# BadgerTechnologies/navigation

Hardware: AMD Instinct MI355X
Metric: scored trajectories/sec (whole node) + costmap inflation cells/sec, 400x400 map (higher is better)
Workload: dtype f64

## Files before the change

include/navgpu.h:

```cpp
#ifndef NAVGPU_H_
#define NAVGPU_H_

#include <stddef.h>
#include <stdint.h>

#ifdef __cplusplus
extern "C" {
#endif

typedef enum {
  NAVGPU_OK = 0,
  NAVGPU_ERR_INVALID = -1,
  NAVGPU_ERR_NO_DEVICE = -2,
  NAVGPU_ERR_HIP = -3,
  NAVGPU_ERR_CAPACITY = -4,
  NAVGPU_ERR_STATE = -5
} navgpu_status;

#define NAVGPU_NO_INFORMATION 255
#define NAVGPU_LETHAL_OBSTACLE 254
#define NAVGPU_INSCRIBED_INFLATED_OBSTACLE 253
#define NAVGPU_FREE_SPACE 0

#define NAVGPU_LAYER_STATIC 1
// ... 151 lines not shown
int navgpu_footprint_from_radius(double radius, double* xy16);
int navgpu_set_footprint(navgpu_fleet* fleet, uint32_t first, uint32_t count, const double* footprint_xy,
                         uint32_t n_vertices);

int navgpu_costmap_stage(navgpu_fleet* fleet, uint32_t first, uint32_t count, const double* robot_poses,
                         const navgpu_observation* observations, uint32_t n_observations,
                         const float* points_xyz, uint32_t n_points_total);
int navgpu_costmap_update(navgpu_fleet* fleet, uint32_t first, uint32_t count);
int navgpu_costmap_bounds(navgpu_fleet* fleet, uint32_t first, uint32_t count, int32_t* boxes);

int navgpu_inflate(navgpu_fleet* fleet, uint32_t first, uint32_t count, const int32_t* boxes);
int navgpu_obstacle_update_bounds(navgpu_fleet* fleet, uint32_t first, uint32_t count, double* bounds_inout);
int navgpu_obstacle_update_costs(navgpu_fleet* fleet, uint32_t first, uint32_t count, const int32_t* boxes);

int navgpu_planner_configure(navgpu_fleet* fleet, const navgpu_dwa_config* config);
int navgpu_planner_set_plan(navgpu_fleet* fleet, uint32_t first, uint32_t count);
int navgpu_planner_stage(navgpu_fleet* fleet, uint32_t first, uint32_t count, const navgpu_robot_state* states,
                         const double* plan_xy, uint32_t n_plan_total);
int navgpu_planner_stage_poses(navgpu_fleet* fleet, uint32_t first, uint32_t count, const float* pos_xyth, const float* vel_xyth);
int navgpu_planner_cycle(navgpu_fleet* fleet, uint32_t first, uint32_t count);
int navgpu_planner_set_bounded_map_grids(navgpu_fleet* fleet, int32_t enable);
int navgpu_planner_set_map_grid_options(navgpu_fleet* fleet, int32_t critic, int32_t aggregation, double yshift);
int navgpu_planner_wavefront_levels(navgpu_fleet* fleet, uint32_t first, uint32_t count, uint32_t* levels);
int navgpu_planner_wavefront_boxes(navgpu_fleet* fleet, uint32_t first, uint32_t count, int32_t* boxes);
int navgpu_planner_results(navgpu_fleet* fleet, uint32_t first, uint32_t count, navgpu_plan_result* results);
int navgpu_planner_set_cycles_in_flight(navgpu_fleet* fleet, int32_t cycles);
int navgpu_planner_results_previous(navgpu_fleet* fleet, uint32_t first, uint32_t count, navgpu_plan_result* results);
int navgpu_planner_trajectory(navgpu_fleet* fleet, uint32_t instance, double* xyth, uint32_t capacity_points);
int navgpu_planner_samples(navgpu_fleet* fleet, uint32_t instance, double* costs, int32_t* status,
                           float* velocities_xyz, uint32_t capacity);
int navgpu_planner_check_trajectory(navgpu_fleet* fleet, uint32_t instance, const float vel_samples[3], int32_t* ok);
int navgpu_planner_check_trajectories(navgpu_fleet* fleet, uint32_t n_robots, const uint32_t* instances,
                                      const uint32_t* probe_offsets , const float* vel_samples ,
                                      int32_t* ok , double* costs );
int navgpu_planner_cost_cloud(navgpu_fleet* fleet, uint32_t instance, float* points, uint32_t capacity);
#define NAVGPU_TRAJ_CLOUD_MAX_ROBOTS 16
int navgpu_planner_set_trajectory_cloud(navgpu_fleet* fleet, uint32_t first, uint32_t count, int32_t enable);
int navgpu_planner_trajectory_cloud(navgpu_fleet* fleet, uint32_t instance, int32_t reference_costs, float* points, uint32_t capacity);
typedef struct {
  double critic[5];
  double cost_full;
  double cost_ref;
  int32_t first_fail;
  int32_t status;
  int32_t n_points;
  int32_t member;
// ... 575 lines not shown
```

navigation_amd/_lib.py:

```python
import ctypes as C
import os
import subprocess

import numpy as np

_HERE = os.path.dirname(os.path.abspath(__file__))
_LIB = None

LAYER_STATIC, LAYER_OBSTACLE, LAYER_VOXEL, LAYER_INFLATION = 1, 2, 4, 8
GRID_MASTER, GRID_STATIC, GRID_OBSTACLE, GRID_VOXEL, GRID_PATH, GRID_GOAL, GRID_GOAL_FRONT = range(7)
OBS_MARKING, OBS_CLEARING = 1, 2
VOXEL_UNKNOWN, VOXEL_MARKED = 1, 2
K_OBSTACLE, K_MERGE, K_INFLATE, K_BFS, K_SCORE, K_SELECT, K_FOOTPRINT, K_VOXEL_EXPORT, K_OBS_INGEST, K_CHECK_TRAJ = range(10)
KERNELS = ("k_obstacle", "k_merge", "k_inflate", "k_bfs", "k_score", "k_select", "k_footprint_cost", "k_voxel_export", "k_obs_ingest", "k_check_traj")
CLOUD_XYZ, CLOUD_SCAN = 0, 1
OBSBUF_MAX_SOURCES, OBSBUF_MAX_CLOUD_POINTS = 8, 65536


class NavgpuError(RuntimeError):
    pass


class FleetDesc(C.Structure):
    _fields_ = [("n_instances", C.c_uint32), ("size_x", C.c_uint32), ("size_y", C.c_uint32),
# ... 414 lines not shown
    ("navgpu_grid_reset", C.c_int, [vp, C.c_int, u32, u32]),
    ("navgpu_grid_reset_window", C.c_int, [vp, C.c_int, u32, u32, u32, u32, u32, u32]),
    ("navgpu_layer_reset_bounding_box", C.c_int, [vp, u32, u32, vp]),
    ("navgpu_static_set_map", C.c_int, [vp, u32, u32, vp, i32, i32, i32, i32, i32]),
    ("navgpu_static_set_rolling_map", C.c_int, [vp, vp, u32, u32, C.c_double, C.c_double, C.c_double, i32, i32, i32, i32, i32]),
    ("navgpu_static_set_transform", C.c_int, [vp, u32, u32, vp]),
    ("navgpu_obstacle_configure", C.c_int, [vp, C.POINTER(ObstacleParams)]),
    ("navgpu_inflation_configure", C.c_int, [vp, C.POINTER(InflationParams)]),
    ("navgpu_set_footprint", C.c_int, [vp, u32, u32, vp, u32]),
    ("navgpu_costmap_stage", C.c_int, [vp, u32, u32, vp, vp, u32, vp, u32]),
    ("navgpu_costmap_update", C.c_int, [vp, u32, u32]),
    ("navgpu_costmap_bounds", C.c_int, [vp, u32, u32, vp]),
    ("navgpu_inflate", C.c_int, [vp, u32, u32, vp]),
    ("navgpu_obstacle_update_bounds", C.c_int, [vp, u32, u32, vp]),
    ("navgpu_obstacle_update_costs", C.c_int, [vp, u32, u32, vp]),
    ("navgpu_planner_configure", C.c_int, [vp, C.POINTER(DwaConfig)]),
    ("navgpu_planner_set_plan", C.c_int, [vp, u32, u32]),
    ("navgpu_planner_stage", C.c_int, [vp, u32, u32, vp, vp, u32]),
    ("navgpu_planner_stage_poses", C.c_int, [vp, u32, u32, vp, vp]),
    ("navgpu_planner_cycle", C.c_int, [vp, u32, u32]),
    ("navgpu_planner_set_bounded_map_grids", C.c_int, [vp, C.c_int32]),
    ("navgpu_planner_set_map_grid_options", C.c_int, [vp, C.c_int32, C.c_int32, C.c_double]),
    ("navgpu_planner_wavefront_levels", C.c_int, [vp, u32, u32, vp]),
    ("navgpu_planner_wavefront_boxes", C.c_int, [vp, u32, u32, vp]),
    ("navgpu_planner_results", C.c_int, [vp, u32, u32, vp]),
    ("navgpu_planner_set_cycles_in_flight", C.c_int, [vp, C.c_int32]),
    ("navgpu_planner_results_previous", C.c_int, [vp, u32, u32, vp]),
    ("navgpu_planner_trajectory", C.c_int, [vp, u32, vp, u32]),
    ("navgpu_planner_samples", C.c_int, [vp, u32, vp, vp, vp, u32]),
    ("navgpu_planner_check_trajectory", C.c_int, [vp, u32, vp, C.POINTER(i32)]),
    ("navgpu_planner_check_trajectories", C.c_int, [vp, u32, vp, vp, vp, vp, vp]),
    ("navgpu_planner_cost_cloud", C.c_int, [vp, u32, vp, u32]),
    ("navgpu_planner_set_trajectory_cloud", C.c_int, [vp, u32, u32, i32]),
    ("navgpu_planner_trajectory_cloud", C.c_int, [vp, u32, i32, vp, u32]),
    ("navgpu_planner_sample_terms", C.c_int, [vp, u32, vp, u32]),
    ("navgpu_planner_get_oscillation", C.c_int, [vp, u32, u32, vp, vp]),
    ("navgpu_planner_set_oscillation", C.c_int, [vp, u32, u32, vp, vp]),
    ("navgpu_local_plan_window", C.c_int, [vp, u32, vp, vp, dbl, i32, vp, u32, C.POINTER(u32), C.POINTER(u32)]),
    ("navgpu_shortest_angular_distance", dbl, [dbl, dbl]),
    ("navgpu_local_planner_configure", C.c_int, [vp, C.POINTER(LocalLimits)]),
    ("navgpu_local_planner_set_plan", C.c_int, [vp, u32, vp, u32, vp]),
    ("navgpu_local_planner_compute_velocity_commands", C.c_int, [vp, u32, u32, vp, vp]),
    ("navgpu_local_planner_is_goal_reached", C.c_int, [vp, u32, u32, vp, vp]),
    ("navgpu_local_planner_get_plan", C.c_int, [vp, u32, vp, u32]),
    ("navgpu_local_planner_reserve_plans", C.c_int, [vp, u32]),
    ("navgpu_local_planner_set_plans", C.c_int, [vp, u32, u32, vp, vp, vp]),
# ... 134 lines not shown
```

navigation_amd/csrc/navgpu_device.h:

```cpp
#pragma once
#include <hip/hip_runtime.h>
#include <stdint.h>

#include "../../include/navgpu.h"

namespace navgpu {

constexpr uint8_t kNoInfo = 255, kLethal = 254, kInscribed = 253, kFree = 0;
constexpr int kMaxFootprint = 32;
constexpr int kCareRows = 128, kCareWords = 4;
#ifndef NAVGPU_SCORE_TAB_THREADS
#define NAVGPU_SCORE_TAB_THREADS 256
#endif
#ifndef NAVGPU_SCORE_TAB_LDS_KB
#define NAVGPU_SCORE_TAB_LDS_KB 14
#endif
#ifndef NAVGPU_SCORE_PREP_THREADS
#define NAVGPU_SCORE_PREP_THREADS 256
#endif
#ifndef NAVGPU_SCORE_THREADS
#define NAVGPU_SCORE_THREADS 256
#endif
#ifdef NAVGPU_DEBUG_SWITCHES
#define NAVGPU_DEBUG_ENV(name) getenv(name)
#else
#define NAVGPU_DEBUG_ENV(name) ((const char*)nullptr)
#endif
constexpr int kScoreThreads = NAVGPU_SCORE_THREADS;

struct InstCostmapState {
  double last_min_x, last_min_y, last_max_x, last_max_y;
  int32_t need_reinflation;
  int32_t static_has_updated_data;
// ... 92 lines not shown
  uint32_t* within;
  uint32_t win;
  uint32_t fp_rcells;
  uint8_t fp_halfw[32];
  uint32_t fp_chunk;
  uint32_t use_tables, tab_steps, tab_nfp, tab_nth;
  int32_t mg_agg[4];
  double mg_yshift[4];
  int32_t mg_generic;
  uint32_t tab_rows;
  uint32_t tab_bytes;
  double tab_dt;
  uint8_t* prep;
  uint32_t prep_stride, prep_bytes;
  double* sample_cost;
  int32_t* sample_status;
  double* part_cost;
  int32_t* part_index;
  int32_t* counters;
  uint32_t* osc_flags;
  float* osc_prev;
  navgpu_plan_result* result;
  double* traj;
};

struct SampleTerms {
  double v[5];
  int32_t first_fail;
  int32_t fail_code;
  int32_t status;
  int32_t n_points;
};
static_assert(sizeof(SampleTerms) == 56, "terms record");
struct TrajCloudDev {
  const SampleTerms* terms;
  navgpu_sample_terms* out;
  uint32_t* totals;
  float* points;
  uint32_t capacity;
  uint32_t slots_per_group;
  double scale[5];
  int32_t reference_costs;
};
void launch_score_terms(const PlannerDev& pl, uint32_t inst, SampleTerms* terms, hipStream_t s);
struct ProbeBatch {
  const uint32_t* instances;
// ... 324 lines not shown
```

navigation_amd/csrc/navgpu_host.cpp:

```cpp
#include "navgpu_fleet.h"

namespace navgpu {
thread_local std::string g_last_error;
}

extern "C" {

const char* navgpu_version(void) { return "navgpu 0.1 (gfx950)"; }
const char* navgpu_strerror(int status) {
  switch (status) {
    case NAVGPU_OK: return "ok";
    case NAVGPU_ERR_INVALID: return "invalid argument";
    case NAVGPU_ERR_NO_DEVICE: return "no usable HIP device (this library has no CPU fallback)";
    case NAVGPU_ERR_HIP: return "HIP runtime error";
    case NAVGPU_ERR_CAPACITY: return "input exceeds a capacity given at fleet creation";
    case NAVGPU_ERR_STATE: return "call sequence violated";
    default: return "unknown status";
  }
}
const char* navgpu_last_error(void) { return g_last_error.c_str(); }
int navgpu_device_count(void) {
  int n = 0;
  if (hipGetDeviceCount(&n) != hipSuccess) return 0;
  return n;
// ... 173 lines not shown
    f->hp_state = reinterpret_cast<navgpu_robot_state*>(h + o_state);
    f->hp_front = reinterpret_cast<double*>(h + o_front);
    f->hp_align = reinterpret_cast<int32_t*>(h + o_align);
    f->hp_reach = reinterpret_cast<uint32_t*>(h + o_reach);
    f->hp_plan_cnt = reinterpret_cast<uint32_t*>(h + o_pcnt);
    f->hp_plan = reinterpret_cast<double*>(h + o_plan);
  }
  A(pl.fp_spec, (size_t)n * kMaxFootprint * 2);
  A(pl.fp_n, n);
  A(pl.axis_count, (size_t)n * 4);
  A(pl.path, (size_t)n * pl.cells);
  A(pl.goal, (size_t)n * pl.cells);
  A(pl.goal_front, (size_t)n * pl.cells);
  if (bfs_scratch_words(cm.nx, cm.ny)) A(pl.bfs_scratch, (size_t)n * bfs_scratch_words(cm.nx, cm.ny));
  pl.bfs_grids = 3;
  pl.within = nullptr;
  A(pl.bfs_box, (size_t)n * 8);
  A(pl.bfs_care, (size_t)n * kCareRows * kCareWords);
  A(pl.bfs_next_item, 4);
  A(pl.bfs_free, (size_t)n * cm.ny * ((cm.nx + 31) / 32));
  A(pl.bfs_levels, (size_t)n * 3);
  A(pl.bfs_order, (size_t)n * 3);
  pl.bfs_bounded = 0;
  A(pl.counters, (size_t)n * 2);
  A(pl.osc_flags, n);
  A(pl.osc_prev, (size_t)n * 3);
  A(pl.traj, (size_t)n * pl.max_sim_steps * 3);
#undef A
  f->h_origin.assign((size_t)n * 2, 0.0);
  f->h_fp_spec.assign((size_t)n * kMaxFootprint * 2, 0.0);
  f->h_fp_n.assign(n, 0);
  f->grid_partial.assign(n, 0);
  f->obs_consumed.assign(n, 0);
  f->bounded_grids = true;
  f->h_box.assign((size_t)n * 4, 0);
  f->inputs_gen.assign(n, 0);
  f->cycle_gen.assign(n, 0);
  launch_fill_u8(cm.master, cm.master_default, (size_t)n * cm.cells_padded, f->stream);
  if (cm.obst) launch_fill_u8(cm.obst, cm.obstacle_default, (size_t)n * cm.cells_padded, f->stream);
  if (cm.voxel) launch_fill_u32(cm.voxel, 0x0000FFFFu, (size_t)n * cm.cells_padded, f->stream);
  std::vector<InstCostmapState> st(n);
  for (auto& s : st) {
    memset(&s, 0, sizeof(s));
    s.last_min_x = -FLT_MAX;
    s.last_min_y = -FLT_MAX;
    s.last_max_x = FLT_MAX;
// ... 825 lines not shown
  if (f->cycles_in_flight > 1) {
    HIP_TRY(hipEventRecord(f->ev_pl_h2d, f->stream));
    f->ev_pl_set = true;
  }
  return NAVGPU_OK;
}

int navgpu_planner_set_bounded_map_grids(navgpu_fleet* f, int32_t enable) {
  if (!f) return NAVGPU_ERR_INVALID;
  FleetGuard guard_(f);
  f->bounded_grids = enable != 0;
  return restageReach(f);
}
int navgpu_planner_set_map_grid_options(navgpu_fleet* f, int32_t critic, int32_t aggregation, double yshift) {
  if (!f || critic < 0 || critic > 3 || aggregation < 0 || aggregation > 2 || !std::isfinite(yshift)) return NAVGPU_ERR_INVALID;
  FleetGuard guard_(f);
  PlannerDev& pl = f->pl;
  pl.mg_agg[critic] = aggregation;
  pl.mg_yshift[critic] = yshift;
  pl.mg_generic = 0;
  for (int k = 0; k < 4; ++k)
    if (pl.mg_agg[k] != 0 || pl.mg_yshift[k] != 0.0) pl.mg_generic = 1;
  return restageReach(f);
}
int navgpu_planner_wavefront_levels(navgpu_fleet* f, uint32_t first, uint32_t count, uint32_t* levels) {
  if (!f || !levels || !f->rangeOk(first, count)) return NAVGPU_ERR_INVALID;
  FleetGuard guard_(f);
  HIP_TRY(hipMemcpyAsync(levels, f->pl.bfs_levels + (size_t)first * 3, sizeof(uint32_t) * 3 * count, hipMemcpyDeviceToHost, f->stream));
  HIP_TRY(waitStream(f->stream));
  return NAVGPU_OK;
}

int navgpu_planner_configure(navgpu_fleet* f, const navgpu_dwa_config* c) {
  if (!f || !c) return NAVGPU_ERR_INVALID;
  FleetGuard guard_(f);
  if (!(c->sim_time > 0) || !(c->sim_granularity > 0) || !(c->angular_sim_granularity > 0)) return NAVGPU_ERR_INVALID;
  PlannerDev& pl = f->pl;
  navgpu_dwa_config cfg = *c;
  if (cfg.vx_samples <= 0) cfg.vx_samples = 1;
  if (cfg.vy_samples <= 0) cfg.vy_samples = 1;
  if (cfg.vth_samples <= 0) cfg.vth_samples = 1;
  if (cfg.rollout_trig != 0 && cfg.rollout_trig != 1) return NAVGPU_ERR_INVALID;
  const uint32_t max_axis = (uint32_t)std::max(std::max(cfg.vx_samples, cfg.vy_samples), std::max(cfg.vth_samples, 2)) + 1;
  if (max_axis > 128) return NAVGPU_ERR_CAPACITY;
  double steps;
  if (cfg.discretize_by_time)
// ... 544 lines not shown
```

navigation_amd/csrc/planner_bfs_common.h:

```cpp
#pragma once
#include "planner_common.h"

namespace navgpu {

template <typename Set>
__device__ __forceinline__ void bfsPlanSeeds(const PlannerDev& pl, const uint32_t inst, const int which, const Geom& g, const uint8_t* master,
                                             const uint32_t nx, const uint32_t tid, uint32_t* s_wave, Set&& set) {
  const uint32_t n = pl.plan_count[inst];
  const double* P = pl.plan + (size_t)inst * pl.max_plan * 2;
  const bool ovr = which == 2;
  const double lx = pl.front_last[2 * inst], ly = pl.front_last[2 * inst + 1];
  const uint32_t chunk = (n + blockDim.x - 1) / blockDim.x;
  const uint32_t i0 = min(n, tid * chunk), i1 = min(n, i0 + chunk);
  uint32_t mine = 0;
  for (uint32_t i = i0; i < i1; ++i) mine += adjustedPoints(P, i, lx, ly, ovr, n, g.res, true, [](uint32_t, double, double) {});
  uint32_t total;
  const uint32_t base = blockExclusiveScan1024(mine, s_wave, &total);
  auto valid = [&](double x, double y, uint32_t& cell) {
    uint32_t mx, my;
    if (!worldToMap(g, x, y, mx, my)) return false;
    cell = my * nx + mx;
    return master[cell] != kNoInfo;
  };
  uint32_t fmin_ = 0xFFFFFFFFu, b = base;
// ... 60 lines not shown
__device__ __forceinline__ uint32_t bfsColMask(const int x0, const int x1, const int j) {
  const int c_lo = max(x0 - j * 32, 0), c_hi = min(x1 - j * 32, 31);
  return c_hi >= c_lo ? ((0xFFFFFFFFu >> (31 - c_hi)) & (0xFFFFFFFFu << c_lo)) : 0u;
}

__device__ __forceinline__ void bfsStoreCells(uint32_t* word_base, uint32_t cells, const uint32_t value, const bool aligned4) {
  if (aligned4) {
    uint32_t full = cells & (cells >> 1) & (cells >> 2) & (cells >> 3) & 0x11111111u;
    cells &= ~(full * 15u);
    const uint4 v4 = make_uint4(value, value, value, value);
    while (full) {
      const uint32_t bpos = (uint32_t)__ffs(full) - 1u;
      *reinterpret_cast<uint4*>(word_base + bpos) = v4;
      full &= full - 1;
    }
  }
  while (cells) {
    const uint32_t bpos = (uint32_t)__ffs(cells) - 1u;
    word_base[bpos] = value;
    cells &= cells - 1;
  }
}

__device__ __forceinline__ void bfsStamp(const PlannerDev& pl, const uint32_t tid, const uint32_t item, const uint32_t slot) {
  if (pl.bfs_trace && tid == 0) pl.bfs_trace[(size_t)item * 8 + slot] = wall_clock64();
}
__device__ __forceinline__ void bfsFinish(const PlannerDev& pl, const uint32_t tid, const uint32_t inst, const int which, const uint32_t item, const uint32_t level) {
  if (pl.bfs_trace && tid == 0) {
    pl.bfs_trace[(size_t)item * 8 + 6] = wall_clock64();
    pl.bfs_trace[(size_t)item * 8 + 1] = wall_clock64() | ((unsigned long long)level << 48);
  }
  if (tid == 0 && pl.bfs_grids == 3) pl.bfs_levels[(size_t)inst * 3 + which] = level;
}

}
```

navigation_amd/csrc/planner_bfs_rows.hip:

```cpp
#include "planner_bfs_common.h"

namespace navgpu {

#ifdef NAVGPU_BFS_STATS
__device__ unsigned long long g_bfs_stats[16];
#define BFS_STAMP(v) const unsigned long long v = __builtin_amdgcn_s_memtime()
#define BFS_ACC(i, x) bst[i] += (x)
#else
#define BFS_STAMP(v)
#define BFS_ACC(i, x)
#endif
#ifndef NAVGPU_ROWS_RECORD_PAD
#define NAVGPU_ROWS_RECORD_PAD 4
#endif
constexpr uint32_t kRowsRecordPad = NAVGPU_ROWS_RECORD_PAD;
template <int W>
__host__ __device__ inline size_t bfs_rows_lds_words(uint32_t nx, uint32_t ny) {
  constexpr uint32_t Wp = (W + 3) & ~3u;
  const uint32_t nw = bfs_rows_waves(ny);
  return (((size_t)nw * kRowsPerWave * ((nx + 31) >> 5) + 3) & ~(size_t)3) + (size_t)kCareRows * kCareWords + (size_t)(nw + 2) * 2 * kRowsHalo * (2 * Wp + kRowsRecordPad);
}
#define NAVGPU_ROWS_DPP " row_mask:0xf bank_mask:0xf bound_ctrl:1\n\t"
#define NAVGPU_ROWS_GROUP_WORDS                                    \
  "v_mov_b32 %[p], %[f3]\n\t"                                      \
// ... 59 lines not shown
               "s_or_b32 %[hi], %[hi], %[st]\n\t"
               "s_cmp_lg_u64 %[c0], 0\n\t"
               "s_cselect_b32 %[st], %[bit], 0\n\t"
               "s_or_b32 %[nz], %[nz], %[st]\n\t"
               "1:\n\t"
               : NAVGPU_ROWS_GROUP_REGS, [nz] "+s"(nz), [lo] "+s"(lo), [hi] "+s"(hi), [c0] "=&s"(c0), [c1] "=&s"(c1), [c2] "=&s"(c2), [st] "=&s"(st)
               : [aw] "s"(aw), [g] "n"(g), [bit] "n"(1 << g), [L] "v"(L), [R] "v"(R)
               : "scc");
}
#undef NAVGPU_ROWS_GROUP_REGS
#undef NAVGPU_ROWS_GROUP_WORDS
#undef NAVGPU_ROWS_DPP
template <int W>
__device__ __forceinline__ void bfsRowsGrid(const PlannerDev& pl, const uint32_t inst, const int which, const uint32_t item) {
  constexpr int NG = (W + 3) / 4;
  constexpr int WP = NG * 4;
  constexpr int D = kRowsHalo;
  const BfsRegion rg = bfsRegion(pl, inst);
  const int bx0 = rg.x0, bx1 = rg.x1, by0 = rg.y0, by1 = rg.y1, care_ok = rg.care_ok;
  extern __shared__ __align__(16) uint32_t sm[];
  __shared__ uint32_t s_wave[16];
  __shared__ uint32_t s_flag[3];
  __shared__ uint32_t s_open[3];
  uint32_t tid_ = threadIdx.x, nx_ = pl.nx, ny_ = pl.ny;
  asm volatile("" : "+v"(tid_), "+s"(nx_), "+s"(ny_));
  const uint32_t tid = tid_;
  bfsStamp(pl, tid, item, 0);
  const Geom g = geomOf(pl, inst);
  const uint32_t nx = nx_, ny = ny_, Wr = (nx + 31) >> 5;
  const uint32_t nw = blockDim.x >> 6;
  const uint32_t lane = tid & 63u, wave_id = tid >> 6;
  const int row_i = (int)(wave_id * kRowsPerWave + lane) - D;
  const bool real = row_i >= 0 && row_i < (int)ny;
  const bool owner = real && lane >= (uint32_t)D && lane < 64u - D;
  const uint32_t row = real ? (uint32_t)row_i : 0u;
  const uint32_t rows_p = nw * kRowsPerWave;
  const uint32_t seed_words = (rows_p * Wr + 3u) & ~3u;
  uint32_t* seedm = sm;
  uint32_t* care_l = sm + seed_words;
  uint32_t* edge = care_l + kCareRows * kCareWords;
  constexpr uint32_t RS = 2 * WP + kRowsRecordPad;
  const uint32_t edge_words = (nw + 2) * 2 * D * RS;
  const uint8_t* master = pl.master + (size_t)inst * pl.cells_padded;
  const uint32_t* freew = bfsFreeBitmap(pl, which, inst, ny * Wr);
  uint32_t* dist = (which == 0 ? pl.path : (which == 1 ? pl.goal : pl.goal_front)) + (size_t)inst * pl.cells;
  const uint32_t N_obst = pl.cells, N_unreach = pl.cells + 1;
  const uint32_t last_mask = (nx & 31) ? ((1u << (nx & 31)) - 1u) : 0xFFFFFFFFu;
  const bool aligned4 = (nx & 3) == 0;

  for (uint32_t i = tid; i < seed_words + kCareRows * kCareWords + edge_words; i += blockDim.x) sm[i] = 0;
  if (tid < 3) s_flag[tid] = s_open[tid] = 0;
  __syncthreads();
  bfsStamp(pl, tid, item, 4);
  if (care_ok) {
    const uint32_t* care = pl.bfs_care + (size_t)inst * kCareRows * kCareWords;
    for (uint32_t i = tid; i < (uint32_t)(kCareRows * kCareWords); i += blockDim.x) care_l[i] = care[i];
  }
  bfsPlanSeeds(pl, inst, which, g, master, nx, tid, s_wave, [&](uint32_t mx, uint32_t my) {
    atomicOr(&seedm[my * Wr + (mx >> 5)], 1u << (mx & 31));
  });
  __syncthreads();
  bfsStamp(pl, tid, item, 5);

  uint32_t blocked[WP], fr[WP];
#pragma unroll
  for (int j = 0; j < WP; ++j) {
    blocked[j] = 0xFFFFFFFFu;
    fr[j] = 0;
    if (real && (uint32_t)j < Wr) {
      fr[j] = seedm[row * Wr + j];
      blocked[j] = ~(freew[row * Wr + j] & ((uint32_t)j + 1 == Wr ? last_mask : 0xFFFFFFFFu)) | fr[j];
    }
  }
  const bool wave_in_box = (int)(wave_id * kRowsPerWave) <= by1 && (int)((wave_id + 1) * kRowsPerWave) > by0;
  const bool row_in_box = owner && row_i >= by0 && row_i <= by1;
  const int w0 = rg.w0, w1 = rg.w1;
  const uint32_t region_groups = bfsRegionGroups(rg);
  uint32_t* drow = dist + (size_t)row * nx;
  auto storeCells = [&](int j, uint32_t cells, uint32_t value) { bfsStoreCells(drow + j * 32, cells, value, aligned4); };
  const bool pub_top = lane >= (uint32_t)D && lane < 2u * D, pub_bot = lane >= 64u - 2 * D && lane < 64u - D;
  const uint32_t pub_wr = (((wave_id + 1) * 2 + (pub_top ? 0u : 1u)) * D + (pub_top ? lane - D : lane - (64u - 2 * D))) * RS;
  const bool halo_top = lane < (uint32_t)D, halo_bot = lane >= 64u - D;
  const uint32_t halo_rd = ((halo_top ? (wave_id * 2 + 1) : ((wave_id + 2) * 2)) * D + (halo_top ? lane : lane - (64u - D))) * RS;
  constexpr uint32_t gmask = (1u << NG) - 1u;

  constexpr bool kBlockLive = W != 20;
  static_assert(D >= 1 && D < 32, "the edge masks take D bits of one word");
  constexpr uint32_t edge_lo = kBlockLive ? (1u << D) - 1u : 0xFFFFFFFFu, edge_hi = kBlockLive ? ~(0xFFFFFFFFu >> D) : 0xFFFFFFFFu;
  auto activity = [&]() -> uint32_t {
    uint32_t nz = 0, lo = 0, hi = 0;
#pragma unroll
    for (int q = 0; q < NG; ++q) {
      const uint32_t t = fr[4 * q] | fr[4 * q + 1] | fr[4 * q + 2] | fr[4 * q + 3];
      if (__builtin_amdgcn_ballot_w64(t != 0) != 0) {
        nz |= 1u << q;
// ... 5 lines not shown
  };
  if (wave_in_box) {
#pragma unroll
    for (int j = 0; j < W; ++j)
      if (j >= w0 && j <= w1 && row_in_box) storeCells(j, fr[j], 0u);
  }
  uint32_t a_own = activity();
  uint32_t level = 0, xch = 0;
  bfsStamp(pl, tid, item, 2);
  bool done = false;
#ifdef NAVGPU_BFS_STATS
  unsigned long long bst[9] = {0, 0, 0, 0, 0, 0, 0, 0, 0};
#endif
  auto storeNew = [&](const uint32_t groups) {
    if (wave_in_box && (groups & region_groups) != 0) {
#pragma unroll
      for (int q = 0; q < NG; ++q) {
        if (((groups & region_groups) >> q) & 1u) {
#pragma unroll
          for (int c = 0; c < 4; ++c) {
            const int j = 4 * q + c;
            if (j < W && j >= w0 && j <= w1) {
#ifndef NAVGPU_BFS_X_NOSTORE
              if (row_in_box && fr[j < W ? j : 0] != 0) storeCells(j, fr[j < W ? j : 0], level + 1);
#endif
            }
          }
        }
      }
    }
  };
  while (!done) {
    bool any_new;
    if constexpr (kBlockLive) {
      const uint32_t aw = __builtin_amdgcn_readfirstlane(a_own);
      uint64_t acc = 0;
      if (aw == 0) {
        BFS_ACC(5, D);
        level += D;
      } else {
        for (int k = 0; k < D; ++k) {
          BFS_STAMP(ts1);
          BFS_ACC(5, 1);
          BFS_ACC(7, 1);
          BFS_ACC(8, __builtin_popcount(aw));
          uint32_t awk = aw;
          asm volatile("" : "+s"(awk));
// ... 71 lines not shown
      s_open[(xch + 1) % 3u] = 0;
    }
    BFS_STAMP(ts5);
    BFS_ACC(3, ts5 - ts4);
    __syncthreads();
    done = !s_flag[slot] || !s_open[slot];
    if (!done) {
      if ((halo_top || halo_bot) && real) {
#pragma unroll
        for (int q = 0; q < WP; q += 4) {
          const uint4 v = *reinterpret_cast<const uint4*>(edge + halo_rd + q);
          const uint4 b = *reinterpret_cast<const uint4*>(edge + halo_rd + WP + q);
          fr[q] = v.x;
          fr[q + 1] = v.y;
          fr[q + 2] = v.z;
          fr[q + 3] = v.w;
          blocked[q] = b.x;
          blocked[q + 1] = b.y;
          blocked[q + 2] = b.z;
          blocked[q + 3] = b.w;
        }
      }
      a_own = activity();
      __syncthreads();
    }
    ++xch;
    BFS_STAMP(ts6);
    BFS_ACC(4, ts6 - ts5);
  }
#ifdef NAVGPU_BFS_STATS
  if (lane == 0)
    for (int k = 0; k < 9; ++k) atomicAdd(&g_bfs_stats[k], bst[k]);
#endif
  bfsStamp(pl, tid, item, 3);

  __syncthreads();
  {
    uint32_t ex[WP], fb[WP];
#pragma unroll
    for (int j = 0; j < WP; ++j) {
      const bool in = owner && (uint32_t)j < Wr;
      fb[j] = in ? (freew[row * Wr + j] & ((uint32_t)j + 1 == Wr ? last_mask : 0xFFFFFFFFu)) : 0u;
      ex[j] = in ? ((blocked[j] & fb[j]) | seedm[row * Wr + j]) : 0u;
    }
    if (pub_top || pub_bot) {
#pragma unroll
// ... 1 lines not shown
    }
    __syncthreads();
    if ((halo_top || halo_bot) && real) {
#pragma unroll
      for (int j = 0; j < WP; ++j) ex[j] = edge[halo_rd + j];
    }
    if (wave_in_box) {
#pragma unroll
      for (int j = 0; j < W; ++j) {
        if (j >= w0 && j <= w1) {
          const uint32_t fc = ex[j];
          const uint32_t lw = j > 0 ? ex[j > 0 ? j - 1 : 0] : 0u, rw = j + 1 < WP ? ex[j + 1 < WP ? j + 1 : 0] : 0u;
          const uint32_t nbr = __builtin_amdgcn_alignbit(fc, lw, 31) | __builtin_amdgcn_alignbit(rw, fc, 1) | fromLaneBelow(fc) | fromLaneAbove(fc);
          const uint32_t cm = (uint32_t)j + 1 == Wr ? last_mask : ((uint32_t)j < Wr ? 0xFFFFFFFFu : 0u);
          const uint32_t touched = nbr & ~fb[j] & ~fc & cm;
          if (row_in_box) {
            storeCells(j, touched, N_obst);
            storeCells(j, ~fc & ~touched & cm, N_unreach);
          }
        }
      }
    }
  }
  bfsFinish(pl, tid, inst, which, item, level);
}
template <int W>
__global__ __launch_bounds__(1024, 6) void k_bfs_rows(PlannerDev pl, uint32_t first, uint32_t count, uint32_t* next_item, const uint32_t* order) {
  __shared__ uint32_t s_item;
  const uint32_t total = count * pl.bfs_grids;
  for (;;) {
    if (threadIdx.x == 0) s_item = atomicAdd(next_item, 1u);
    __syncthreads();
    const uint32_t slot = s_item;
    if (slot >= total) break;
    const uint32_t item = order ? order[slot] : slot;
    const uint32_t g = item / count;
    bfsRowsGrid<W>(pl, first + (item - g * count), (int)pl.bfs_grids - 1 - (int)g, item);
    __syncthreads();
  }
}
constexpr int kRows2HaloLanes = 4;
constexpr int kRows2Levels = 2 * kRows2HaloLanes;
constexpr int kRows2PerWave = 2 * (64 - 2 * kRows2HaloLanes);
constexpr int kRows2Words = 32;
__host__ __device__ inline uint32_t bfs_rows2_waves(uint32_t ny) { return (ny + kRows2PerWave - 1) / kRows2PerWave; }
__host__ __device__ inline size_t bfs_rows2_lds_words(uint32_t ny) {
  return (size_t)kCareRows * kCareWords + (size_t)(bfs_rows2_waves(ny) + 2) * 2 * kRows2HaloLanes * 4 * kRows2Words;
// ... 459 lines not shown
```

navigation_amd/csrc/planner_samples.hip:

```cpp
#include "planner_common.h"

namespace navgpu {

constexpr int kSamplesThreads = 128;
__global__ __launch_bounds__(kSamplesThreads) void k_samples(PlannerDev pl, uint32_t first, uint32_t count) {
  const uint32_t tid = threadIdx.x & 63u, wv = threadIdx.x >> 6;
  if (blockIdx.x >= 2 * count) {
    const uint32_t W = (pl.nx + 31) >> 5, words = pl.ny * W, per = (words + kSamplesThreads - 1) / kSamplesThreads;
    const uint32_t b = blockIdx.x - 2 * count, r = b / per, i = (b - r * per) * kSamplesThreads + threadIdx.x;
    if (i < words) {
      const uint32_t row = i / W, wi = i - row * W;
      pl.bfs_free[(size_t)(first + r) * words + i] = bfsFreeWord(pl.master + (size_t)(first + r) * pl.cells_padded, row, pl.nx, wi, pl.cfg.allow_unknown != 0 ? 0u : 1u);
    }
    return;
  }
  const navgpu_dwa_config& c = pl.cfg;
  if (blockIdx.x >= count) {
    const uint32_t robot = blockIdx.x - count, inst = first + robot;
    if (wv == 0) {
      const uint32_t total = 3 * count;
      uint32_t key[3], before[3] = {0, 0, 0};
#pragma unroll
      for (uint32_t g = 0; g < 3; ++g) key[g] = pl.bfs_levels[(size_t)inst * 3 + (2 - g)];
#pragma unroll 4
      for (uint32_t j = tid; j < total; j += 64) {
        const uint32_t gj = j / count, rj = j - gj * count;
        const uint32_t kj = pl.bfs_levels[(size_t)(first + rj) * 3 + (2 - gj)];
#pragma unroll
        for (uint32_t g = 0; g < 3; ++g) before[g] += (kj > key[g] || (kj == key[g] && j < g * count + robot)) ? 1u : 0u;
      }
#pragma unroll
      for (uint32_t g = 0; g < 3; ++g)
        for (int o = 32; o > 0; o >>= 1) before[g] += __shfl_xor(before[g], o);
      if (tid < 3) pl.bfs_order[(size_t)first * 3 + (tid == 0 ? before[0] : (tid == 1 ? before[1] : before[2]))] = tid * count + robot;
      if (robot == 0 && tid < 2) pl.bfs_next_item[tid] = 0;
      return;
    }
    const navgpu_robot_state st = pl.state[inst];
    int32_t* cnt = pl.axis_count + 4 * inst;
    int n = 0;
    if (tid < 3) {
      const int a = tid;
      const float vsamp = a == 0 ? (float)c.vx_samples : (a == 1 ? (float)c.vy_samples : (float)c.vth_samples);
      const double max_vel_th = c.max_rot_vel, min_vel_th = -1.0 * max_vel_th;
      double lim_min = a == 0 ? c.min_vel_x : (a == 1 ? c.min_vel_y : min_vel_th);
      double lim_max = a == 0 ? c.max_vel_x : (a == 1 ? c.max_vel_y : max_vel_th);
      const float acc = a == 0 ? (float)c.acc_lim_x : (a == 1 ? (float)c.acc_lim_y : (float)c.acc_lim_theta);
      const float v = st.vel[a];
      float maxv, minv;
      if (!c.use_dwa) {
// ... 208 lines not shown
```

navigation_amd/fleet.py:

```python
import ctypes as C

import numpy as np

from . import _lib as N
from ._lib import (DwaConfig, FleetDesc, InflationParams, NavgpuError, Observation, ObstacleParams, PlanResult,
                   RobotState, check, lib)

_GRID_DTYPE = {N.GRID_MASTER: np.uint8, N.GRID_STATIC: np.uint8, N.GRID_OBSTACLE: np.uint8,
               N.GRID_VOXEL: np.uint32, N.GRID_PATH: np.uint32, N.GRID_GOAL: np.uint32,
               N.GRID_GOAL_FRONT: np.uint32}


def _ptr(a):
    return a.ctypes.data_as(C.c_void_p)


class Fleet:
    def __init__(self, n_instances, size_x, size_y, resolution, layers=N.LAYER_OBSTACLE | N.LAYER_INFLATION,
                 track_unknown=False, device=0, max_points=1024, max_observations=4, max_plan=256,
                 max_footprint=16, max_sim_steps=64, keep_sample_costs=False, rolling_window=False):
        self.L = lib()
        d = FleetDesc(n_instances, size_x, size_y, resolution, layers, int(track_unknown), device, max_points,
                      max_observations, max_plan, max_footprint, max_sim_steps, int(keep_sample_costs), int(rolling_window))
        self.desc = d
# ... 289 lines not shown

    def wavefront_boxes(self, first=0, count=None):
        first, count = self._range(first, count)
        out = np.zeros((count, 4), np.int32)
        check(self.L.navgpu_planner_wavefront_boxes(self.h, first, count, _ptr(out)), "wavefront_boxes")
        return out

    MAP_GRID_CRITICS = {"path": 0, "goal": 1, "goal_front": 2, "alignment": 3}
    AGGREGATIONS = {"last": 0, "sum": 1, "product": 2}

    def set_map_grid_options(self, critic, aggregation="last", yshift=0.0):
        check(self.L.navgpu_planner_set_map_grid_options(self.h, self.MAP_GRID_CRITICS[critic], self.AGGREGATIONS[aggregation], float(yshift)),
              "set_map_grid_options")

    def set_bounded_map_grids(self, enable):
        check(self.L.navgpu_planner_set_bounded_map_grids(self.h, 1 if enable else 0), "set_bounded_map_grids")

    def wavefront_levels(self, first=0, count=None):
        first, count = self._range(first, count)
        out = np.zeros((count, 3), np.uint32)
        check(self.L.navgpu_planner_wavefront_levels(self.h, first, count, _ptr(out)), "wavefront_levels")
        return out

    def planner_cycle(self, first=0, count=None):
        first, count = self._range(first, count)
        check(self.L.navgpu_planner_cycle(self.h, first, count), "planner_cycle")

    def results(self, first=0, count=None):
        first, count = self._range(first, count)
        r = (PlanResult * count)()
        check(self.L.navgpu_planner_results(self.h, first, count, C.cast(r, C.c_void_p)), "planner_results")
        return list(r)

    def results_into(self, buf, first=0):
        check(self.L.navgpu_planner_results(self.h, first, len(buf), C.cast(buf, C.c_void_p)), "planner_results")
        return buf

    def set_cycles_in_flight(self, cycles):
        check(self.L.navgpu_planner_set_cycles_in_flight(self.h, int(cycles)), "set_cycles_in_flight")

    def results_previous_into(self, buf, first=0):
        check(self.L.navgpu_planner_results_previous(self.h, first, len(buf), C.cast(buf, C.c_void_p)), "planner_results_previous")
        return buf

    def find_best_path(self, pos, vel, plans, first=0):
        pos = np.ascontiguousarray(pos, np.float32).reshape(-1, 3)
# ... 390 lines not shown
```

Measured before the change: 6.293 billion.

## Resume planner wavefront BFS from cached mid-level snapshots across cycles

Stores a per-instance, per-grid snapshot of the row-bitset BFS frontier and visited mask at a chosen level, outside the region that changed since the last cycle. On later cycles with the same single seed and no free-space changes outside the guarded box, the BFS restarts from that snapshot level instead of from the seed, which skips the early levels. Level counts used for work ordering are adjusted by the resumed offset. It adds snapshot memory, extra validation passes and global writes, and its correctness depends on how well the changed-region tracking works.

```diff
diff --git a/include/navgpu.h b/include/navgpu.h
--- a/include/navgpu.h
+++ b/include/navgpu.h
@@ -197,6 +197,8 @@
 int navgpu_planner_set_bounded_map_grids(navgpu_fleet* fleet, int32_t enable);
 int navgpu_planner_set_map_grid_options(navgpu_fleet* fleet, int32_t critic, int32_t aggregation, double yshift);
 int navgpu_planner_wavefront_levels(navgpu_fleet* fleet, uint32_t first, uint32_t count, uint32_t* levels);
+int navgpu_planner_set_wavefront_resume(navgpu_fleet* fleet, int32_t enable);
+int navgpu_planner_wavefront_resumed(navgpu_fleet* fleet, uint32_t first, uint32_t count, uint32_t* l0);
 int navgpu_planner_wavefront_boxes(navgpu_fleet* fleet, uint32_t first, uint32_t count, int32_t* boxes);
 int navgpu_planner_results(navgpu_fleet* fleet, uint32_t first, uint32_t count, navgpu_plan_result* results);
 int navgpu_planner_set_cycles_in_flight(navgpu_fleet* fleet, int32_t cycles);
diff --git a/navigation_amd/_lib.py b/navigation_amd/_lib.py
--- a/navigation_amd/_lib.py
+++ b/navigation_amd/_lib.py
@@ -460,6 +460,8 @@
     ("navgpu_planner_set_bounded_map_grids", C.c_int, [vp, C.c_int32]),
     ("navgpu_planner_set_map_grid_options", C.c_int, [vp, C.c_int32, C.c_int32, C.c_double]),
     ("navgpu_planner_wavefront_levels", C.c_int, [vp, u32, u32, vp]),
+    ("navgpu_planner_set_wavefront_resume", C.c_int, [vp, C.c_int32]),
+    ("navgpu_planner_wavefront_resumed", C.c_int, [vp, u32, u32, vp]),
     ("navgpu_planner_wavefront_boxes", C.c_int, [vp, u32, u32, vp]),
     ("navgpu_planner_results", C.c_int, [vp, u32, u32, vp]),
     ("navgpu_planner_set_cycles_in_flight", C.c_int, [vp, C.c_int32]),
diff --git a/navigation_amd/csrc/navgpu_device.h b/navigation_amd/csrc/navgpu_device.h
--- a/navigation_amd/csrc/navgpu_device.h
+++ b/navigation_amd/csrc/navgpu_device.h
@@ -9,6 +9,8 @@
 constexpr uint8_t kNoInfo = 255, kLethal = 254, kInscribed = 253, kFree = 0;
 constexpr int kMaxFootprint = 32;
 constexpr int kCareRows = 128, kCareWords = 4;
+constexpr uint32_t kSnapSlots = 2, kSnapMetaWords = 12;
+__host__ __device__ inline size_t bfsSnapSlotWords(uint32_t nx, uint32_t ny) { return (size_t)3 * ny * ((nx + 31) >> 5); }
 #ifndef NAVGPU_SCORE_TAB_THREADS
 #define NAVGPU_SCORE_TAB_THREADS 256
 #endif
@@ -147,6 +149,11 @@
   float* osc_prev;
   navgpu_plan_result* result;
   double* traj;
+  uint32_t* bfs_snap;
+  uint32_t* bfs_snap_meta;
+  uint32_t* bfs_resumed;
+  const InstCostmapState* cm_state;
+  uint32_t bfs_resume;
 };
 
 struct SampleTerms {
diff --git a/navigation_amd/csrc/navgpu_host.cpp b/navigation_amd/csrc/navgpu_host.cpp
--- a/navigation_amd/csrc/navgpu_host.cpp
+++ b/navigation_amd/csrc/navgpu_host.cpp
@@ -219,6 +219,13 @@
   A(pl.bfs_levels, (size_t)n * 3);
   A(pl.bfs_order, (size_t)n * 3);
   pl.bfs_bounded = 0;
+  if (!bfs_scratch_words(cm.nx, cm.ny)) {
+    A(pl.bfs_snap, (size_t)n * 2 * kSnapSlots * bfsSnapSlotWords(cm.nx, cm.ny));
+    A(pl.bfs_snap_meta, (size_t)n * 2 * kSnapSlots * kSnapMetaWords);
+  }
+  A(pl.bfs_resumed, (size_t)n * 3);
+  pl.cm_state = cm.state;
+  pl.bfs_resume = 1;
   A(pl.counters, (size_t)n * 2);
   A(pl.osc_flags, n);
   A(pl.osc_prev, (size_t)n * 3);
@@ -1090,6 +1097,19 @@
   for (int k = 0; k < 4; ++k)
     if (pl.mg_agg[k] != 0 || pl.mg_yshift[k] != 0.0) pl.mg_generic = 1;
   return restageReach(f);
+}
+int navgpu_planner_set_wavefront_resume(navgpu_fleet* f, int32_t enable) {
+  if (!f) return NAVGPU_ERR_INVALID;
+  FleetGuard guard_(f);
+  f->pl.bfs_resume = enable != 0 ? 1u : 0u;
+  return NAVGPU_OK;
+}
+int navgpu_planner_wavefront_resumed(navgpu_fleet* f, uint32_t first, uint32_t count, uint32_t* l0) {
+  if (!f || !l0 || !f->rangeOk(first, count)) return NAVGPU_ERR_INVALID;
+  FleetGuard guard_(f);
+  HIP_TRY(hipMemcpyAsync(l0, f->pl.bfs_resumed + (size_t)first * 3, sizeof(uint32_t) * 3 * count, hipMemcpyDeviceToHost, f->stream));
+  HIP_TRY(waitStream(f->stream));
+  return NAVGPU_OK;
 }
 int navgpu_planner_wavefront_levels(navgpu_fleet* f, uint32_t first, uint32_t count, uint32_t* levels) {
   if (!f || !levels || !f->rangeOk(first, count)) return NAVGPU_ERR_INVALID;
diff --git a/navigation_amd/csrc/planner_bfs_common.h b/navigation_amd/csrc/planner_bfs_common.h
--- a/navigation_amd/csrc/planner_bfs_common.h
+++ b/navigation_amd/csrc/planner_bfs_common.h
@@ -106,6 +106,30 @@
   }
 }
 
+enum : uint32_t { kSnapValid = 0, kSnapSeed = 1, kSnapL0 = 2, kSnapG = 3 , kSnapStamp = 7, kSnapStreak = 8  };
+constexpr uint32_t kSnapBetterCycles = 8;
+constexpr int kSnapMargin = 8;
+__device__ __forceinline__ uint32_t* bfsSnapMeta(const PlannerDev& pl, const uint32_t inst, const int which, const uint32_t slot) {
+  return pl.bfs_snap_meta + (((size_t)inst * 2 + (uint32_t)(which - 1)) * kSnapSlots + slot) * kSnapMetaWords;
+}
+__device__ __forceinline__ uint32_t* bfsSnapBits(const PlannerDev& pl, const uint32_t inst, const int which, const uint32_t slot) {
+  return pl.bfs_snap + (((size_t)inst * 2 + (uint32_t)(which - 1)) * kSnapSlots + slot) * bfsSnapSlotWords(pl.nx, pl.ny);
+}
+struct BfsBox {
+  int x0, x1, y0, y1;
+  __device__ __forceinline__ void include(int a0, int a1, int b0, int b1) {
+    x0 = min(x0, a0);
+    x1 = max(x1, a1);
+    y0 = min(y0, b0);
+    y1 = max(y1, b1);
+  }
+  __device__ __forceinline__ bool holds(int a0, int a1, int b0, int b1) const { return a0 >= x0 && a1 <= x1 && b0 >= y0 && b1 <= y1; }
+};
+__device__ __forceinline__ uint32_t bfsResumeLevel(const BfsBox& g, const int sx, const int sy) {
+  const int d = max(max(g.x0 - sx, sx - g.x1), 0) + max(max(g.y0 - sy, sy - g.y1), 0);
+  return d >= kRowsHalo + 2 ? (uint32_t)((d - 2) / kRowsHalo * kRowsHalo) : 0u;
+}
+
 __device__ __forceinline__ void bfsStamp(const PlannerDev& pl, const uint32_t tid, const uint32_t item, const uint32_t slot) {
   if (pl.bfs_trace && tid == 0) pl.bfs_trace[(size_t)item * 8 + slot] = wall_clock64();
 }
diff --git a/navigation_amd/csrc/planner_bfs_rows.hip b/navigation_amd/csrc/planner_bfs_rows.hip
--- a/navigation_amd/csrc/planner_bfs_rows.hip
+++ b/navigation_amd/csrc/planner_bfs_rows.hip
@@ -105,6 +105,7 @@
   __shared__ uint32_t s_wave[16];
   __shared__ uint32_t s_flag[3];
   __shared__ uint32_t s_open[3];
+  __shared__ uint32_t s_snap[22];
   uint32_t tid_ = threadIdx.x, nx_ = pl.nx, ny_ = pl.ny;
   asm volatile("" : "+v"(tid_), "+s"(nx_), "+s"(ny_));
   const uint32_t tid = tid_;
@@ -130,9 +131,11 @@
   const uint32_t N_obst = pl.cells, N_unreach = pl.cells + 1;
   const uint32_t last_mask = (nx & 31) ? ((1u << (nx & 31)) - 1u) : 0xFFFFFFFFu;
   const bool aligned4 = (nx & 3) == 0;
+  const bool snap_on_ = pl.bfs_resume != 0 && pl.bfs_snap != nullptr && pl.bfs_bounded != 0 && pl.bfs_grids == 3 && which >= 1 && rg.bounded;
 
   for (uint32_t i = tid; i < seed_words + kCareRows * kCareWords + edge_words; i += blockDim.x) sm[i] = 0;
   if (tid < 3) s_flag[tid] = s_open[tid] = 0;
+  if (tid < 22) s_snap[tid] = (tid == 4 || tid == 6 || tid == 19) ? 0xFFFFFFFFu : (tid == 21 && snap_on_ ? 1u : 0u);
   __syncthreads();
   bfsStamp(pl, tid, item, 4);
   if (care_ok) {
@@ -141,10 +144,105 @@
   }
   bfsPlanSeeds(pl, inst, which, g, master, nx, tid, s_wave, [&](uint32_t mx, uint32_t my) {
     atomicOr(&seedm[my * Wr + (mx >> 5)], 1u << (mx & 31));
+    if (s_snap[21] != 0) {
+      atomicAdd(&s_snap[0], 1u);
+      s_snap[1] = my * nx + mx;
+    }
   });
   __syncthreads();
   bfsStamp(pl, tid, item, 5);
 
+  if (__builtin_amdgcn_readfirstlane(s_snap[21]) != 0) {
+    if (tid == 0 && s_snap[0] == 1u) {
+      const uint32_t seedc = s_snap[1];
+      const uint32_t* m0 = bfsSnapMeta(pl, inst, which, 0);
+      const uint32_t* m1 = m0 + kSnapMetaWords;
+      const bool v0 = m0[kSnapValid] != 0, v1 = m1[kSnapValid] != 0;
+      const bool hit0 = v0 && m0[kSnapSeed] == seedc, hit1 = v1 && m1[kSnapSeed] == seedc;
+      const uint32_t t = hit0 ? 0u : (hit1 ? 1u : (!v0 ? 0u : (!v1 ? 1u : (m0[kSnapStamp] <= m1[kSnapStamp] ? 0u : 1u))));
+      const uint32_t* mt = t ? m1 : m0;
+      s_snap[8] = t;
+      s_snap[9] = mt[kSnapValid];
+      for (int k = 0; k < 4; ++k) s_snap[10 + k] = mt[kSnapG + k];
+      s_snap[14] = 1;
+      s_snap[15] = (hit0 || hit1) ? 1u : 0u;
+      s_snap[16] = mt[kSnapL0];
+      s_snap[17] = max(m0[kSnapStamp], m1[kSnapStamp]) + 1u;
+      s_snap[20] = mt[kSnapStreak];
+    }
+    __syncthreads();
+    if (s_snap[14] != 0) {
+      const uint32_t words = ny * Wr;
+      if (s_snap[9] != 0 && owner) {
+        uint32_t ro = row * Wr;
+        asm volatile("" : "+v"(ro));
+        const uint32_t* then = bfsSnapBits(pl, inst, which, s_snap[8]) + 2 * words + ro;
+        const int gx0 = (int)s_snap[10], gx1 = (int)s_snap[11];
+        const bool row_in_g = row_i >= (int)s_snap[12] && row_i <= (int)s_snap[13];
+        uint32_t lo = 0xFFFFFFFFu, hi = 0, bad = 0;
+#pragma unroll 1
+        for (uint32_t j = 0; j < Wr; ++j) {
+          const uint32_t d = (freew[ro + j] ^ then[j]) & (j + 1 == Wr ? last_mask : 0xFFFFFFFFu);
+          if (d != 0) {
+            lo = min(lo, j * 32 + (uint32_t)__ffs(d) - 1u);
+            hi = max(hi, j * 32 + 31u - (uint32_t)__clz(d));
+            bad |= row_in_g ? (d & ~bfsColMask(gx0, gx1, (int)j)) : d;
+          }
+        }
+        if (lo <= hi) {
+          atomicMin(&s_snap[4], lo);
+          atomicMax(&s_snap[5], hi);
+          atomicMin(&s_snap[6], row);
+          atomicMax(&s_snap[7], row);
+          if (bad != 0) s_snap[2] = 1;
+        }
+      }
+      if (owner && row_i >= by0 && row_i <= by1) {
+        uint32_t open_any = 0;
+        const uint32_t rr = (uint32_t)(row_i - by0);
+        uint32_t ro = row * Wr;
+        asm volatile("" : "+v"(ro));
+#pragma unroll 1
+        for (int j = rg.w0; j <= rg.w1; ++j) {
+          const uint32_t cw_i = (uint32_t)(j - rg.w0);
+          const uint32_t care = (care_ok != 0 && cw_i < (uint32_t)kCareWords && rr < (uint32_t)kCareRows) ? care_l[rr * kCareWords + cw_i] : (care_ok ? 0u : 0xFFFFFFFFu);
+          const uint32_t fw = (uint32_t)j < Wr ? (freew[ro + j] & ((uint32_t)j + 1 == Wr ? last_mask : 0xFFFFFFFFu)) : 0u;
+          open_any |= fw & care & bfsColMask(bx0, bx1, j);
+        }
+        if (open_any != 0) s_snap[3] = 1;
+      }
+    }
+    __syncthreads();
+    if (tid == 0 && s_snap[14] != 0) {
+      const uint32_t seedc = s_snap[1];
+      uint32_t* mt = bfsSnapMeta(pl, inst, which, s_snap[8]);
+      const BfsBox tg{(int)s_snap[10], (int)s_snap[11], (int)s_snap[12], (int)s_snap[13]};
+      BfsBox gn{bx0, bx1, by0, by1};
+      const InstCostmapState& cs = pl.cm_state[inst];
+      if (cs.box_valid) gn.include(cs.box[0], cs.box[1] - 1, cs.box[2], cs.box[3] - 1);
+      if (s_snap[4] <= s_snap[5]) gn.include((int)s_snap[4], (int)s_snap[5], (int)s_snap[6], (int)s_snap[7]);
+      gn = BfsBox{max(gn.x0 - kSnapMargin, 0), min(gn.x1 + kSnapMargin, (int)nx - 1), max(gn.y0 - kSnapMargin, 0), min(gn.y1 + kSnapMargin, (int)ny - 1)};
+      const uint32_t l0_now = bfsResumeLevel(gn, (int)(seedc % nx), (int)(seedc / nx)), t_l0 = s_snap[16];
+      const bool usable = s_snap[15] != 0 && s_snap[2] == 0 && tg.holds(bx0, bx1, by0, by1);
+      const uint32_t streak = (usable && t_l0 + 2u * D < l0_now) ? s_snap[20] + 1u : 0u;
+      if (usable && streak < kSnapBetterCycles) {
+        if (s_snap[3] != 0) s_snap[18] = t_l0;
+        mt[kSnapStamp] = s_snap[17];
+        mt[kSnapStreak] = streak;
+      } else if (l0_now != 0) {
+        s_snap[19] = l0_now;
+        s_snap[10] = (uint32_t)gn.x0;
+        s_snap[11] = (uint32_t)gn.x1;
+        s_snap[12] = (uint32_t)gn.y0;
+        s_snap[13] = (uint32_t)gn.y1;
+      } else if (s_snap[9] != 0) {
+        mt[kSnapValid] = 0;
+      }
+    }
+    __syncthreads();
+  }
+  const uint32_t resume_l0 = __builtin_amdgcn_readfirstlane(s_snap[18]);
+  if (tid == 0 && pl.bfs_bounded != 0 && pl.bfs_grids == 3 && pl.bfs_resumed != nullptr) pl.bfs_resumed[(size_t)inst * 3 + which] = resume_l0;
   uint32_t blocked[WP], fr[WP];
 #pragma unroll
   for (int j = 0; j < WP; ++j) {
@@ -154,6 +252,20 @@
       fr[j] = seedm[row * Wr + j];
       blocked[j] = ~(freew[row * Wr + j] & ((uint32_t)j + 1 == Wr ? last_mask : 0xFFFFFFFFu)) | fr[j];
     }
+  }
+  if (resume_l0 != 0 && real) {
+    uint32_t ro = row * Wr, words = ny * Wr, wr = Wr, lm = last_mask;
+    unsigned long long sb = (unsigned long long)bfsSnapBits(pl, inst, which, __builtin_amdgcn_readfirstlane(s_snap[8]));
+    asm volatile("" : "+v"(ro), "+v"(words), "+v"(wr), "+v"(lm), "+v"(sb));
+    const uint32_t* snap = reinterpret_cast<const uint32_t*>(sb) + ro;
+    const uint32_t* fnow = freew + ro;
+#pragma unroll
+    for (int j = 0; j < WP; ++j)
+      if ((uint32_t)j < wr) {
+        fr[j] = snap[j];
+        blocked[j] = ~(fnow[j] & ((uint32_t)j + 1 == wr ? lm : 0xFFFFFFFFu)) | snap[words + j];
+        asm volatile("" ::: "memory");
+      }
   }
   const bool wave_in_box = (int)(wave_id * kRowsPerWave) <= by1 && (int)((wave_id + 1) * kRowsPerWave) > by0;
   const bool row_in_box = owner && row_i >= by0 && row_i <= by1;
@@ -205,7 +317,7 @@
             const int j = 4 * q + c;
             if (j < W && j >= w0 && j <= w1) {
 #ifndef NAVGPU_BFS_X_NOSTORE
-              if (row_in_box && fr[j < W ? j : 0] != 0) storeCells(j, fr[j < W ? j : 0], level + 1);
+              if (row_in_box && fr[j < W ? j : 0] != 0) storeCells(j, fr[j < W ? j : 0], resume_l0 + level + 1);
 #endif
             }
           }
@@ -323,6 +435,34 @@
         }
       }
       a_own = activity();
+      if (resume_l0 + level == s_snap[19]) {
+        uint32_t ro = row * Wr, words = ny * Wr, wr = Wr, lm = last_mask;
+        unsigned long long sb = (unsigned long long)bfsSnapBits(pl, inst, which, __builtin_amdgcn_readfirstlane(s_snap[8]));
+        asm volatile("" : "+v"(ro), "+v"(words), "+v"(wr), "+v"(lm), "+v"(sb));
+        uint32_t* snap = reinterpret_cast<uint32_t*>(sb) + ro;
+        const uint32_t* fnow = freew + ro;
+        const uint32_t* seeds = seedm + ro;
+        if (owner) {
+#pragma unroll
+          for (int j = 0; j < WP; ++j)
+            if ((uint32_t)j < wr) {
+              const uint32_t fw = fnow[j] & ((uint32_t)j + 1 == wr ? lm : 0xFFFFFFFFu);
+              snap[j] = fr[j];
+              snap[words + j] = (blocked[j] & fw) | seeds[j];
+              snap[2 * words + j] = fw;
+              asm volatile("" ::: "memory");
+            }
+        }
+        if (tid == 0) {
+          uint32_t* m = bfsSnapMeta(pl, inst, which, s_snap[8]);
+          m[kSnapValid] = 1;
+          m[kSnapSeed] = s_snap[1];
+          m[kSnapL0] = resume_l0 + level;
+          for (int k = 0; k < 4; ++k) m[kSnapG + k] = s_snap[10 + k];
+          m[kSnapStamp] = s_snap[17];
+          m[kSnapStreak] = 0;
+        }
+      }
       __syncthreads();
     }
     ++xch;
@@ -370,7 +510,7 @@
       }
     }
   }
-  bfsFinish(pl, tid, inst, which, item, level);
+  bfsFinish(pl, tid, inst, which, item, resume_l0 + level);
 }
 template <int W>
 __global__ __launch_bounds__(1024, 6) void k_bfs_rows(PlannerDev pl, uint32_t first, uint32_t count, uint32_t* next_item, const uint32_t* order) {
diff --git a/navigation_amd/csrc/planner_samples.hip b/navigation_amd/csrc/planner_samples.hip
--- a/navigation_amd/csrc/planner_samples.hip
+++ b/navigation_amd/csrc/planner_samples.hip
@@ -3,6 +3,10 @@
 namespace navgpu {
 
 constexpr int kSamplesThreads = 128;
+__device__ __forceinline__ uint32_t bfsItemLevels(const PlannerDev& pl, const uint32_t inst, const uint32_t which) {
+  const uint32_t lv = pl.bfs_levels[(size_t)inst * 3 + which], l0 = pl.bfs_resumed[(size_t)inst * 3 + which];
+  return lv > l0 ? lv - l0 : 0u;
+}
 __global__ __launch_bounds__(kSamplesThreads) void k_samples(PlannerDev pl, uint32_t first, uint32_t count) {
   const uint32_t tid = threadIdx.x & 63u, wv = threadIdx.x >> 6;
   if (blockIdx.x >= 2 * count) {
@@ -21,11 +25,11 @@
       const uint32_t total = 3 * count;
       uint32_t key[3], before[3] = {0, 0, 0};
 #pragma unroll
-      for (uint32_t g = 0; g < 3; ++g) key[g] = pl.bfs_levels[(size_t)inst * 3 + (2 - g)];
+      for (uint32_t g = 0; g < 3; ++g) key[g] = bfsItemLevels(pl, inst, 2 - g);
 #pragma unroll 4
       for (uint32_t j = tid; j < total; j += 64) {
         const uint32_t gj = j / count, rj = j - gj * count;
-        const uint32_t kj = pl.bfs_levels[(size_t)(first + rj) * 3 + (2 - gj)];
+        const uint32_t kj = bfsItemLevels(pl, first + rj, 2 - gj);
 #pragma unroll
         for (uint32_t g = 0; g < 3; ++g) before[g] += (kj > key[g] || (kj == key[g] && j < g * count + robot)) ? 1u : 0u;
       }
diff --git a/navigation_amd/fleet.py b/navigation_amd/fleet.py
--- a/navigation_amd/fleet.py
+++ b/navigation_amd/fleet.py
@@ -335,6 +335,15 @@
         check(self.L.navgpu_planner_wavefront_levels(self.h, first, count, _ptr(out)), "wavefront_levels")
         return out
 
+    def set_wavefront_resume(self, enable):
+        check(self.L.navgpu_planner_set_wavefront_resume(self.h, 1 if enable else 0), "set_wavefront_resume")
+
+    def wavefront_resumed(self, first=0, count=None):
+        first, count = self._range(first, count)
+        out = np.zeros((count, 3), np.uint32)
+        check(self.L.navgpu_planner_wavefront_resumed(self.h, first, count, _ptr(out)), "wavefront_resumed")
+        return out
+
     def planner_cycle(self, first=0, count=None):
         first, count = self._range(first, count)
         check(self.L.navgpu_planner_cycle(self.h, first, count), "planner_cycle")
```

Result: no change. 6.355 billion, median of 6 (+1.0%).
